# RmSchaffert/ACCV-Lab

Measured on AMD Instinct MI355X. Metric: heatmap frames/sec (1920x1080 fp32, ragged N_obj in [1,128], fused clear+draw), higher is better.
Workload: dtype f32

## Files before the change

### accv-lab_amd/accvlab/_amd_native/__init__.py

```python
from __future__ import annotations

import ctypes
import os

_HERE = os.path.dirname(os.path.abspath(__file__))
NO_HOST_FASTPATH = os.environ.get("ACCV_NO_HOST_FASTPATH", "") not in ("", "0")
LIB_PATH = os.environ.get("ACCV_HIP_LIB") or os.path.join(_HERE, "libaccv_hip.so")

OK = 0
HM_CLEAR = 1
HM_COUNTS_I64 = 2
HM_SMALL_RADII = 4
HM_WRITE_THROUGH = 8
HM_GROUP_BOXES_GIVEN = 16
HM_TILE_ROWS_16 = 32
HM_TILE_ROWS_8 = 64
HM_CALLER_SCALE_ORDER = 256
HM_PLAIN_STORES = 128
HM_POINT_COUNTS_I64 = 512
MP_IDX_I64 = 1
MP_COUNTS_I64 = 2
MP_LABELS_I64 = 4
FL_AVG_NUM_POS = 0
FL_AVG_VALUE = 1
FL_AVG_DEVICE = 2
LSA_MAXIMIZE = 1
LSA_THREADS_64 = 2
LSA_THREADS_1024 = 4
MC_ONE_MINUS_PROB = 0
MC_NEG_PROB = 1
MC_FOCAL = 2
MC_LABELS_I64 = 1
MC_CXCYWH = 2
CR_MAX_MAPS = 8
CR_MAX_CHANNELS = 64
CR_COUNTS_I64 = 1
CR_INDEX_FORM = 2
CR_WEIGHTS_PER_CHANNEL = 4
CR_L1 = 0
CR_SMOOTH_L1 = 2
MF_IDX_I64 = 1
MF_LABELS_I64 = 2
MB_IDX_I64 = 1
MB_CXCYWH = 2
MB_IOU_NONE = 0
MB_IOU = 1
MB_GIOU = 2
MB_MAX_D = 16

_vp = ctypes.c_void_p
_i = ctypes.c_int
_f = ctypes.c_float
_u = ctypes.c_uint
_sz = ctypes.c_size_t
_i64 = ctypes.c_int64
_ll = ctypes.c_longlong
_u64 = ctypes.c_uint64

SIGNATURES = {
    "accv_last_error": (ctypes.c_char_p, []),
    "accv_version": (_i, []),
    "accv_draw_heatmap_last_dispatch": (ctypes.c_char_p, []),
    "accv_draw_heatmap_time_next_launch": (_i, [_vp, _vp]),
    "accv_draw_heatmap_flat_workspace_bytes": (_sz, [_i, _i]),
    "accv_draw_heatmap_flat_f32": (_i, [_vp, _i, _i, _i, _vp, _vp, _vp, _i, _f, _f, _u, _vp, _sz, _vp]),
    "accv_draw_heatmap_batched_f32": (_i, [_vp, _i, _i, _i, _i, _vp, _vp, _vp, _vp, _i, _f, _f, _u, _vp]),
    "accv_fill_f32": (_i, [_vp, _sz, _f, _vp]),
    "accv_draw_heatmap_multiscale_f32": (_i, [_vp, _vp, _vp, _vp, _i, _i, _vp, _vp, _vp, _i, _f, _f, _u, _vp]),
    "accv_draw_heatmap_multiscale_sample_f32": (_i, [_vp, _vp, _vp, _vp, _i, _i, _vp, _vp, _vp, _i, _f, _f, _u,
                                                      _vp, _i, _i, _vp, _i, _vp, _vp, _vp]),
    "accv_draw_points_workspace_bytes": (_sz, [_i, _i]),
    "accv_draw_points_multiscale_f32": (_i, [_vp, _vp, _vp, _vp, _i, _i, _vp, _vp, _i, _i, _f, _f, _u, _vp, _sz, _vp]),
# ... 246 lines not shown
```

### accv-lab_amd/accvlab/draw_heatmap/ops.py

```python
from __future__ import annotations

import ctypes
from typing import Optional

import torch

from .. import _amd_native as _nat

try:
    from . import _dh_host as _dh
except ImportError:
    _dh = None
_native_bound = False


def _native():
    global _native_bound
    if _dh is None or _nat.NO_HOST_FASTPATH:
        return None
    if not _native_bound:
        h = _nat.ctypes_lib()
        addr = lambda name: ctypes.cast(getattr(h, name), ctypes.c_void_p).value
        _dh.bind_native(addr("accv_draw_heatmap_batched_f32"), addr("accv_last_error"))
        _native_bound = True
    return _dh


_FORCED_FLAGS = 0


def _hint_flags(clear: bool, small_radii: bool, write_through: bool, tile_rows) -> int:
    if tile_rows not in (None, 8, 16):
        raise RuntimeError("tile_rows must be None, 8 or 16")
    return (_nat.HM_CLEAR if clear else 0) | (_nat.HM_SMALL_RADII if small_radii else 0) | \
        (0 if write_through is None else _nat.HM_WRITE_THROUGH if write_through else _nat.HM_PLAIN_STORES) | \
        (_nat.HM_TILE_ROWS_16 if tile_rows == 16 else _nat.HM_TILE_ROWS_8 if tile_rows == 8 else 0) | _FORCED_FLAGS


def _one_launch_maps(maps, batch: int, device):
    k = len(maps)
    if not 1 <= k <= 4:
        return None
    ptrs, hs, ws = [], [], []
    for hm in maps:
        if not (isinstance(hm, torch.Tensor) and hm.is_cuda and hm.dtype == torch.float32 and hm.is_contiguous() and
                hm.device == device):
            return None
        shape = hm.shape
        if len(shape) != 3 or shape[0] != batch:
            return None
        ptr = hm.data_ptr()
        if shape[2] % 4 or ptr % 16 or shape[1] * shape[2] * 4 >= (1 << 31):
            return None
        ptrs.append(ptr)
        hs.append(shape[1])
        ws.append(shape[2])
    return (ctypes.c_void_p * k)(*ptrs), (ctypes.c_int * k)(*hs), (ctypes.c_int * k)(*ws)


def _check_maps(maps, batch: int, device, owner: str) -> None:
    for hm in maps:
        _check_input(hm, "heatmap")
        _check_dtype(hm, torch.float32, "heatmap")
        if not (hm.dim() == 3 and hm.size(0) == batch):
            raise RuntimeError("every heatmap must be of shape [batch_size, height, width]")
        if not (hm.device == device):
            raise RuntimeError(f"every heatmap must be on the {owner}' device ({device})")


def _require(cond: bool, msg: str) -> None:
    if not cond:
        raise RuntimeError(msg)


def _check_input(t: torch.Tensor, name: str) -> None:
    if not (isinstance(t, torch.Tensor)):
        raise RuntimeError(f"{name} must be a torch.Tensor")
    if not (t.is_cuda):
        raise RuntimeError(f"{name} must be a CUDA tensor")
    if not (t.is_contiguous()):
        raise RuntimeError(f"{name} must be contiguous")


def _check_dtype(t: torch.Tensor, dtype: torch.dtype, name: str) -> None:
    if not (t.dtype == dtype):
        raise RuntimeError(f"{name}: expected scalar type {dtype} but found {t.dtype}")


def _same_device(ref: torch.Tensor, *others) -> None:
# ... 46 lines not shown
    _check_input(heatmap_idxes, "heatmap_idxes")
    if not (centers.size(0) == radii.size(0)):
        raise RuntimeError("centers and radii must have the same size at dim0")
    if not (centers.size(0) == heatmap_idxes.size(0)):
        raise RuntimeError("centers and heatmap_idxes must have the same size at dim0")
    if not (heatmaps.dim() == 3):
        raise RuntimeError("heatmap must be of shape [num_heatmaps, height, width]")
    if not (centers.dim() == 2 and centers.size(1) == 2):
        raise RuntimeError("centers must be of shape [num_targets, 2]")
    if not (radii.dim() == 1 and heatmap_idxes.dim() == 1):
        raise RuntimeError("radii and heatmap_idxes must be of shape [num_targets]")
    _check_dtype(heatmaps, torch.float32, "heatmap")
    _check_dtype(centers, torch.int32, "centers")
    _check_dtype(radii, torch.int32, "radii")
    _check_dtype(heatmap_idxes, torch.int32, "heatmap_idxes")
    _same_device(heatmaps, ("centers", centers), ("radii", radii), ("heatmap_idxes", heatmap_idxes))

    lib = _nat.lib()
    planes, height, width = heatmaps.shape
    n = centers.size(0)
    if _flat_direct(planes, height, width, n):
        with _nat.device_guard(heatmaps.device):
            dev = heatmaps.device
            count = _device_constant(("count", n, dev), lambda: torch.full((1,), n, dtype=torch.int32, device=dev))
            status = lib.accv_draw_heatmap_batched_f32(
                heatmaps.data_ptr(), 1, planes, height, width, centers.data_ptr(), radii.data_ptr(), count.data_ptr(),
                heatmap_idxes.data_ptr(), n, float(diameter_to_sigma_factor), float(k_scale),
                _hint_flags(clear, small_radii, write_through, tile_rows), _nat.stream_ptr(heatmaps.device))
        _nat.check(status, "draw_heatmap")
        return
    with _nat.device_guard(heatmaps.device):
        ws_bytes = lib.accv_draw_heatmap_flat_workspace_bytes(planes, n)
        ws = torch.empty(ws_bytes, dtype=torch.uint8, device=heatmaps.device)
        status = lib.accv_draw_heatmap_flat_f32(
            heatmaps.data_ptr(), planes, height, width, centers.data_ptr(), radii.data_ptr(),
            heatmap_idxes.data_ptr(), n, float(diameter_to_sigma_factor), float(k_scale),
            _hint_flags(clear, small_radii, write_through, tile_rows), ws.data_ptr(), ws_bytes,
            _nat.stream_ptr(heatmaps.device))
    _nat.check(status, "draw_heatmap")


def draw_heatmap_batched(
    heatmap: torch.Tensor,
    centers,
    radii,
    diameter_to_sigma_factor: float = 6.0,
    k_scale: float = 1.0,
    labels=None,
    *,
    clear: bool = False,
    small_radii: bool = False,
    write_through: Optional[bool] = None,
    tile_rows: Optional[int] = None,
) -> None:
    centers_t = centers.tensor
    radii_t = radii.tensor
    assert centers_t.shape[0] == radii_t.shape[0], "centers and radii must have the same size batch size"
    assert centers_t.shape[1] == radii_t.shape[1], "centers and radii must have the same maximum number of objects"
    counts = centers.sample_sizes
    labels_t: Optional[torch.Tensor] = None
    if labels is not None:
        labels_t = labels.tensor
        assert centers_t.shape[0] == labels_t.shape[0], "centers and labels must have the same size batch size"
        assert centers_t.shape[1] == labels_t.shape[1], \
            "centers and labels must have the same maximum number of objects"

    native = _native()
    if native is not None and isinstance(heatmap, torch.Tensor) and isinstance(counts, torch.Tensor) and \
            native.draw_batched(heatmap, centers_t, radii_t, counts, labels_t, float(diameter_to_sigma_factor), float(k_scale),
                                _hint_flags(clear, small_radii, write_through, tile_rows)):
        return

    if counts.dtype not in (torch.int32, torch.int64):
        counts = counts.to(torch.int64)

    _check_input(heatmap, "heatmap")
    _check_input(centers_t, "centers")
    _check_input(radii_t, "radii")
    _check_input(counts, "nums_targets")
    batch = heatmap.size(0)
    n_max = radii_t.size(1) if radii_t.dim() >= 2 else -1
    _require(batch == radii_t.size(0) and batch == centers_t.size(0) and batch == counts.size(0),
             "batch_size (dim 0) need to be the same for all inputs")
    if not (centers_t.dim() == 3 and centers_t.size(2) == 2):
        raise RuntimeError("centers must be of shape [batch_size, num_targets, 2]")
    if not (radii_t.dim() == 2):
        raise RuntimeError("radii must be of shape [batch_size, num_targets]")
    if not (n_max == centers_t.size(1)):
        raise RuntimeError("maximum number of targets (dim 1) need to be the same centers and radii")
    if not (counts.dim() == 1):
        raise RuntimeError("nums_targets must be of shape [batch_size]")
    _check_dtype(heatmap, torch.float32, "heatmap")
    _check_dtype(centers_t, torch.int32, "centers")
    _check_dtype(radii_t, torch.int32, "radii")
    others = [("centers", centers_t), ("radii", radii_t), ("nums_targets", counts)]
    if labels_t is None:
        if not (heatmap.dim() == 3):
            raise RuntimeError("heatmap must be of shape [batch_size, height, width]")
        num_classes, (height, width) = 0, heatmap.shape[1:]
        labels_ptr = None
    else:
        _check_input(labels_t, "labels")
        if not (heatmap.dim() == 4):
            raise RuntimeError("heatmap must be of shape [batch_size, max_num_classes, height, width]")
        if not (labels_t.dim() == 2):
            raise RuntimeError("labels must be of shape [batch_size, radii.size(1)]")
        _require(labels_t.size(0) == batch and labels_t.size(1) == n_max,
                 "labels shape must be [batch_size, radii.size(1)]")
        _check_dtype(labels_t, torch.int32, "labels")
        num_classes, height, width = heatmap.shape[1:]
        if not (num_classes > 0 or heatmap.numel() == 0):
            raise RuntimeError("class-wise heatmap needs at least one class plane")
        labels_ptr = labels_t.data_ptr()
        others.append(("labels", labels_t))
    _same_device(heatmap, *others)
    if labels_t is not None and num_classes == 0:
        return

    flags = _hint_flags(clear, small_radii, write_through, tile_rows) | \
        (_nat.HM_COUNTS_I64 if counts.dtype == torch.int64 else 0)
    with _nat.device_guard(heatmap.device):
        status = _nat.lib().accv_draw_heatmap_batched_f32(
            heatmap.data_ptr(), batch, num_classes, height, width, centers_t.data_ptr(), radii_t.data_ptr(),
            counts.data_ptr(), labels_ptr, n_max, float(diameter_to_sigma_factor), float(k_scale), flags,
            _nat.stream_ptr(heatmap.device))
    _nat.check(status, "draw_heatmap_batched")


def get_centers_and_radii(centers, bboxes, out_size_factor: float):
    ragged = hasattr(centers, "tensor") and hasattr(centers, "create_with_sample_sizes_like_self")
    c_t = centers.tensor if ragged else centers
    b_t = bboxes.tensor if hasattr(bboxes, "tensor") else bboxes
    _require(c_t.shape[-1] == 2 and b_t.shape[-1] == 4 and c_t.shape[:-1] == b_t.shape[:-1],
             "centers must be [..., 2] and bboxes [..., 4] with equal leading dimensions")
    if c_t.is_cuda:
        if not (b_t.device == c_t.device):
            raise RuntimeError("centers and bboxes must be on the same device")
        c32 = c_t.to(torch.float32).contiguous()
        b32 = b_t.to(torch.float32).contiguous()
        out_c = torch.empty(c32.shape, dtype=torch.int32, device=c32.device)
        out_r = torch.empty(c32.shape[:-1], dtype=torch.int32, device=c32.device)
        with _nat.device_guard(c32.device):
            _nat.check(_nat.lib().accv_heatmap_targets_from_boxes_f32(
                c32.data_ptr(), b32.data_ptr(), out_r.numel(), float(out_size_factor), out_c.data_ptr(),
                out_r.data_ptr(), _nat.stream_ptr(c32.device)), "get_centers_and_radii")
    else:
        d = torch.cat([c_t - b_t[..., :2], b_t[..., 2:] - c_t], dim=-1)
        out_r = torch.ceil(torch.min(d, dim=-1)[0] / out_size_factor).to(torch.int32).clamp_(min=1)
        out_c = (c_t / out_size_factor).to(torch.int32)
    if ragged:
        nu = centers.non_uniform_dim
        return centers.create_with_sample_sizes_like_self(out_c, nu), centers.create_with_sample_sizes_like_self(out_r, nu)
    return out_c, out_r


def draw_heatmap_multiscale(heatmaps, centers, bboxes, out_size_factors, diameter_to_sigma_factor: float = 6.0,
                            k_scale: float = 1.0, *, clear: bool = False) -> None:
    heatmaps = list(heatmaps)
    strides = [float(f) for f in out_size_factors]
    if not (len(heatmaps) == len(strides) and len(heatmaps) >= 1):
        raise RuntimeError("heatmaps and out_size_factors must have the same, non-zero length")
    objects = _box_objects(centers, bboxes)
    batch, dev = objects[0].size(0), objects[0].device
    geometry = _one_launch_maps(heatmaps, batch, dev)
    if geometry is None:
        _check_maps(heatmaps, batch, dev, "centers")
        for hm, f in zip(heatmaps, strides):
            ci, ri = get_centers_and_radii(centers, bboxes, f)
            draw_heatmap_batched(hm, ci, ri, diameter_to_sigma_factor, k_scale, clear=clear)
        return
    _launch_box_maps(geometry, strides, objects, diameter_to_sigma_factor, k_scale, clear)

# ... 43 lines not shown
```

### accv-lab_amd/csrc/draw_heatmap.hip

```cpp
#include <hip/hip_runtime.h>
#include <hip/hip_ext.h>

#include <algorithm>
#include <atomic>
#include <climits>
#include <cstdint>
#include <cstring>
#include <type_traits>

#include "accv_common.h"
#include "polyline_arith.h"

namespace {

constexpr int kWavesPerGroup = 1;
constexpr int kBoxTileR = 8;
constexpr int kCand = 64;
constexpr float kLog2e = 1.4426950408889634f;

struct SplatParams {
    float* hm;
    const int32_t* centers;
    const int32_t* radii;
    const int32_t* labels;
    const void* counts;
    const int32_t* plane_off;
    int H, W;
    int n_max;
    int n_classes;
    int tiles_x, tiles_y;
    long long n_tiles;
    float factor, k;
    int counts_i64;
    int grid3d;
    float dense_area;
    const float* centers_f;
    const float* boxes_f;
    float stride;
    int radius, n_groups;
};

constexpr int kMaxScales = 4;
struct MultiParams {
    SplatParams scale[kMaxScales];
    long long tile_begin[kMaxScales + 1];
    int n_scales;
};

struct __attribute__((aligned(16))) Hit {
    int x, y;
    float c2;
    unsigned box;
};

template <int PX>
struct Vec;
typedef float vfloat4 __attribute__((ext_vector_type(4)));
template <>
struct Vec<4> {
    using type = vfloat4;
};
template <>
struct Vec<1> {
    using type = float;
};

__device__ __forceinline__ float raw_exp2(float x) { return __builtin_amdgcn_exp2f(x); }

__device__ __forceinline__ float max_skip_nan(float acc, float v)
{
    float r;
    asm("v_max_f32 %0, %1, %2" : "=v"(r) : "v"(acc), "v"(v));
    return r;
}

struct TileCtx {
    int tx0, ty0, tx1, ty1;
    long long plane;
    const int2* centers2;
    const int32_t* radii;
    const int32_t* labels;
    const float2* centers_f;
    const float4* boxes_f;
    float4 box0;
    float stride;
    int radius;
    int n, cls;
};
// ... 100 lines not shown
        return Cand{(int)__fdiv_rn(c.x, t.stride), (int)__fdiv_rn(c.y, t.stride), t.radius, 0};
    } else {
        const int2 cxy = t.centers2[cc];
        return Cand{cxy.x, cxy.y, t.radii[cc], t.labels[cc]};
    }
}
__device__ __forceinline__ unsigned long long cull_test(const TileCtx& t, int base, int lane, const Cand& c)
{
    constexpr int kClampXY = 1 << 29, kClampR = 1 << 30;
    const int xc = min(max(c.x, -kClampXY), kClampXY), yc = min(max(c.y, -kClampXY), kClampXY);
    const int rc = min(c.r, kClampR);
    const bool hit = (base + lane < t.n) && (t.cls < 0 || c.label == t.cls) && c.r >= 0 && xc - rc < t.tx1 &&
                     xc + rc >= t.tx0 && yc - rc < t.ty1 && yc + rc >= t.ty0;
    return __ballot(hit);
}
template <int SRC = 0>
__device__ __forceinline__ unsigned long long cull_round(const TileCtx& t, int base, int lane, int& x, int& y, int& r)
{
    const Cand c = cull_load<SRC>(t, base, lane);
    x = c.x;
    y = c.y;
    r = c.r;
    return cull_test(t, base, lane, c);
}

__device__ __forceinline__ float hit_exponent_scale(const SplatParams& p, int r)
{
    const float sigma = (float)(2 * r + 1) / p.factor;
    return kLog2e / (2.0f * sigma * sigma);
}
__device__ __forceinline__ Hit make_hit(const SplatParams& p, const TileCtx& t, int x, int y, int r, float c2);
__device__ __forceinline__ Hit make_hit(const SplatParams& p, const TileCtx& t, int x, int y, int r)
{
    return make_hit(p, t, x, y, r, hit_exponent_scale(p, r));
}
__device__ __forceinline__ Hit make_hit(const SplatParams& p, const TileCtx& t, int x, int y, int r, float c2)
{
    const long long x0 = (long long)x - min(x, r), x1 = (long long)x + min((long long)p.W - x, (long long)r + 1);
    const long long y0 = (long long)y - min(y, r), y1 = (long long)y + min((long long)p.H - y, (long long)r + 1);
    const long long xlo = max(x0, (long long)t.tx0) - t.tx0, xhi = min(x1, (long long)t.tx1) - t.tx0;
    const long long ylo = max(y0, (long long)t.ty0) - t.ty0, yhi = min(y1, (long long)t.ty1) - t.ty0;
    unsigned box = 0;
    if (xhi > xlo && yhi > ylo) box = (unsigned)xlo | ((unsigned)xhi << 8) | ((unsigned)ylo << 16) | ((unsigned)yhi << 24);
    return Hit{x, y, c2, box};
}

__device__ __forceinline__ float max3_skip_nan(float acc, float a, float b)
{
    float r;
    asm("v_max3_f32 %0, %1, %2, %3" : "=v"(r) : "v"(acc), "v"(a), "v"(b));
    return r;
}

template <int PX, int R, bool CLEAR, int SM, int WPG, int SRC>
__device__ __forceinline__ void splat_body(const SplatParams& p, long long linear_group)
{
    constexpr int kWavesPerGroup = WPG;
    constexpr int TW = 32 * PX;
    constexpr int TH = 2 * R;
    static_assert(R % 4 == 0, "row registers are fetched four at a time");

    __shared__ Hit s_hit[kWavesPerGroup][kCand];
    __shared__ __attribute__((aligned(16))) float s_ey[kWavesPerGroup][kCand][TH];

    const int lane = threadIdx.x & 63;
    const int wave = __builtin_amdgcn_readfirstlane(threadIdx.x >> 6);
    TileCtx t;
    if (!locate_tile<TW, TH, kWavesPerGroup>(p, wave, t, linear_group)) return;
    const int tx0 = t.tx0, ty0 = t.ty0, n = t.n;
    const long long plane = t.plane;

    const int sub = lane >> 5;
    const int col0 = tx0 + (lane & 31) * PX;

    float acc[R][PX];
    const float init = CLEAR ? 0.0f : __builtin_nanf("");
#pragma unroll
    for (int i = 0; i < R; ++i)
#pragma unroll
        for (int c = 0; c < PX; ++c) acc[i][c] = init;

    int total_hits = 0;
    float cover = 0.0f;

    for (int base = 0; base < n; base += kCand) {
        int x, y, r;
        const unsigned long long m = cull_round<SRC>(t, base, lane, x, y, r);
        if constexpr (SM == 5) {
            const float dia = (float)(2 * min(max(r, 0), 1 << 20) + 1);
            cover += (base + lane < n) ? dia * dia : 0.0f;
        }
        const bool hit = (m >> lane) & 1ull;
        const int nh = __popcll(m);
        if (nh == 0) continue;
        if constexpr (!CLEAR) {
            if (total_hits == 0 && col0 < p.W) {
                const float* plane_rd = p.hm + (size_t)plane * (size_t)p.H * (size_t)p.W;
#pragma unroll
                for (int i = 0; i < R; ++i) {
                    const int row = ty0 + sub * R + i;
                    if (row < p.H) {
                        if constexpr (PX == 4) {
                            const vfloat4 o = *reinterpret_cast<const vfloat4*>(plane_rd + (size_t)row * p.W + col0);
                            acc[i][0] = o.x;
                            acc[i][1] = o.y;
                            acc[i][2] = o.z;
                            acc[i][3] = o.w;
                        } else {
                            acc[i][0] = plane_rd[(size_t)row * p.W + col0];
                        }
                    }
                }
            }
        }
        if (hit) s_hit[wave][__popcll(m & ((1ull << lane) - 1ull))] = make_hit(p, t, x, y, r);
        __builtin_amdgcn_fence(__ATOMIC_RELEASE, "wavefront");
        __builtin_amdgcn_fence(__ATOMIC_ACQUIRE, "wavefront");

        for (int t = lane; t < nh * TH; t += 64) {
            const int h = t / TH, rr = t % TH;
            const Hit hy = s_hit[wave][h];
            const float d = (float)(ty0 + rr - hy.y);
            const float v = p.k * raw_exp2(-(d * d) * hy.c2);
            const unsigned ylo = (hy.box >> 16) & 255u, yhi = hy.box >> 24;
            s_ey[wave][h][rr] = ((unsigned)rr >= ylo && (unsigned)rr < yhi) ? v : __builtin_nanf("");
        }
        __builtin_amdgcn_fence(__ATOMIC_RELEASE, "wavefront");
        __builtin_amdgcn_fence(__ATOMIC_ACQUIRE, "wavefront");

        const unsigned colr0 = (unsigned)(lane & 31) * PX;
        auto column_factors = [&](const Hit& hx, float (&ex)[PX]) {
            const unsigned xlo = hx.box & 255u, xhi = (hx.box >> 8) & 255u;
#pragma unroll
            for (int c = 0; c < PX; ++c) {
                const float d = (float)(col0 + c - hx.x);
                const float e = raw_exp2(-(d * d) * hx.c2);
                ex[c] = (colr0 + c >= xlo && colr0 + c < xhi) ? e : __builtin_nanf("");
            }
        };
        int h = 0;
        for (; CLEAR && h + 1 < nh; h += 2) {
            float exa[PX], exb[PX];
            column_factors(s_hit[wave][h], exa);
            column_factors(s_hit[wave][h + 1], exb);
#pragma unroll
            for (int q = 0; q < R / 4; ++q) {
                const float4 a4 = *reinterpret_cast<const float4*>(&s_ey[wave][h][sub * R + 4 * q]);
                const float4 b4 = *reinterpret_cast<const float4*>(&s_ey[wave][h + 1][sub * R + 4 * q]);
                const float eya[4] = {a4.x, a4.y, a4.z, a4.w}, eyb[4] = {b4.x, b4.y, b4.z, b4.w};
#pragma unroll
                for (int i = 0; i < 4; ++i)
#pragma unroll
                    for (int c = 0; c < PX; ++c)
                        acc[4 * q + i][c] = max3_skip_nan(acc[4 * q + i][c], exa[c] * eya[i], exb[c] * eyb[i]);
            }
        }
        for (; h < nh; ++h) {
            float ex[PX];
            column_factors(s_hit[wave][h], ex);
#pragma unroll
            for (int q = 0; q < R / 4; ++q) {
                const float4 e4 = *reinterpret_cast<const float4*>(&s_ey[wave][h][sub * R + 4 * q]);
                const float ey[4] = {e4.x, e4.y, e4.z, e4.w};
#pragma unroll
                for (int i = 0; i < 4; ++i)
#pragma unroll
                    for (int c = 0; c < PX; ++c) acc[4 * q + i][c] = max_skip_nan(acc[4 * q + i][c], ex[c] * ey[i]);
            }
        }
        total_hits += nh;
        __builtin_amdgcn_fence(__ATOMIC_RELEASE, "wavefront");
        __builtin_amdgcn_fence(__ATOMIC_ACQUIRE, "wavefront");
    }

    if (!CLEAR && total_hits == 0) return;
    if (col0 >= p.W) return;

    using V = typename Vec<PX>::type;
    float* plane_ptr = p.hm + (size_t)plane * (size_t)p.H * (size_t)p.W;
    bool write_through = SM == 4;
    if constexpr (SM == 5 && PX == 4) {
#pragma unroll
        for (int d = 32; d >= 1; d >>= 1) cover += __shfl_xor(cover, d);
        write_through = cover >= p.dense_area;
    }
#pragma unroll
    for (int i = 0; i < R; ++i) {
        const int row = ty0 + sub * R + i;
        if (row >= p.H) break;
        V* dst = reinterpret_cast<V*>(plane_ptr + (size_t)row * p.W + col0);
        V out;
        if constexpr (PX == 4)
            out = V{acc[i][0], acc[i][1], acc[i][2], acc[i][3]};
        else
            out = acc[i][0];
        if constexpr (SM >= 4 && PX == 4) {
            if (write_through) {
                const auto rsrc = __builtin_amdgcn_make_buffer_rsrc(plane_ptr, 0, (int)((size_t)p.H * p.W * 4), 0x00020000);
                __builtin_amdgcn_raw_buffer_store_b128(out, rsrc, (int)(((size_t)row * p.W + col0) * 4), 0, 18);
            } else {
                *dst = out;
            }
        } else {
            *dst = out;
        }
    }
}

template <int PX, int R, bool CLEAR, int SM, int WPG = kWavesPerGroup>
__global__ __launch_bounds__(WPG * 64) void splat_kernel(const SplatParams p)
{
    splat_body<PX, R, CLEAR, SM, WPG, 0>(p, blockIdx.x);
}

__device__ __forceinline__ int scale_of_group(const MultiParams& mp, long long group, long long& first)
{
    int s = 0;
    first = 0;
#pragma unroll
    for (int i = 1; i < kMaxScales; ++i) {
        const long long begin = mp.tile_begin[i];
        if (group >= begin) {
            s = i;
            first = begin;
        }
    }
    return s;
}
template <typename T>
__device__ __forceinline__ void pin_scalar(T& v)
{
    asm volatile("" : "+s"(v));
}
__device__ __forceinline__ SplatParams preload_params(const SplatParams& src)
{
    SplatParams p = src;
    asm volatile("" ::"s"(p.hm), "s"(p.counts), "s"(p.centers_f), "s"(p.boxes_f));
    pin_scalar(p.H);
    pin_scalar(p.W);
    pin_scalar(p.n_max);
    pin_scalar(p.n_classes);
    pin_scalar(p.tiles_x);
    pin_scalar(p.tiles_y);
    pin_scalar(p.n_tiles);
    pin_scalar(p.factor);
    pin_scalar(p.k);
    pin_scalar(p.counts_i64);
    pin_scalar(p.grid3d);
    pin_scalar(p.dense_area);
    pin_scalar(p.stride);
    pin_scalar(p.radius);
    pin_scalar(p.n_groups);
    return p;
}

template <bool CLEAR, int SM>
__global__ __launch_bounds__(64) void splat_multi_kernel(const MultiParams mp)
{
    long long first;
    const int s = scale_of_group(mp, blockIdx.x, first);
    splat_body<4, kBoxTileR, CLEAR, SM, 1, 1>(mp.scale[s], (long long)blockIdx.x - first);
}

constexpr int kSmallTW = 128, kSmallTH = 16;
constexpr int kSmallLdsW = kSmallTW + 4;
// ... 43 lines not shown
                __hip_atomic_fetch_max(&tile[ylo + py][xlo + px], v, __ATOMIC_RELAXED,
                                       WG_SCOPE ? __HIP_MEMORY_SCOPE_WORKGROUP : __HIP_MEMORY_SCOPE_WAVEFRONT);
            }
        }
    }
    __builtin_amdgcn_fence(__ATOMIC_RELEASE, "wavefront");
    __builtin_amdgcn_fence(__ATOMIC_ACQUIRE, "wavefront");
}
template <bool WG_SCOPE>
__device__ __forceinline__ int splat_round(const SplatParams& p, const TileCtx& t, int lane, unsigned long long m, const Cand& cand,
                                           Hit* __restrict__ hits, SmallTile tile, int rows_hint = 0)
{
    const int nh = __popcll(m);
    int rows = 0;
    if ((m >> lane) & 1ull) {
        const Hit mine = make_hit(p, t, cand.x, cand.y, cand.r);
        hits[__popcll(m & ((1ull << lane) - 1ull))] = mine;
        rows = (int)(mine.box >> 24) - (int)((mine.box >> 16) & 255u);
    }
    if (rows_hint == 0) {
#pragma unroll
        for (int d = 32; d >= 1; d >>= 1) rows = max(rows, __shfl_xor(rows, d));
        rows_hint = max(1, __builtin_amdgcn_readfirstlane(rows));
    }
    walk_hits<WG_SCOPE>(p, t, lane, nh, hits, tile, rows_hint);
    return nh;
}

struct GroupBox {
    float x0, y0, x1, y1;
    bool valid;
};
template <bool FIRST = false>
__device__ __forceinline__ GroupBox load_group_box(const SplatParams& p, const TileCtx& t, int g)
{
    float4 v = FIRST ? t.box0 : t.boxes_f[min(g, p.n_groups - 1)];
    asm volatile("" : "+v"(v.x), "+v"(v.y), "+v"(v.z), "+v"(v.w));
    return GroupBox{v.x, v.y, v.z, v.w, g < p.n_groups && g * kCand < t.n && v.x <= v.z};
}
struct ReachBounds {
    float xlo, xhi, ylo, yhi;
};
__device__ __forceinline__ ReachBounds reach_bounds(const TileCtx& t, int rc, int cx0, int cx1, int cy0, int cy1)
{
    const float r1 = (float)min(rc, 1 << 24) + 2.0f;
    return ReachBounds{((float)cx0 - r1) * t.stride, ((float)cx1 + r1) * t.stride, ((float)cy0 - r1) * t.stride,
                       ((float)cy1 + r1) * t.stride};
}
__device__ __forceinline__ bool group_reaches(const GroupBox& b, const ReachBounds& rb)
{
    return b.valid && b.x1 >= rb.xlo && b.x0 < rb.xhi && b.y1 >= rb.ylo && b.y0 < rb.yhi;
}

constexpr int kDppQuad0 = 0x00, kDppQuad1 = 0x55, kDppQuad2 = 0xAA, kDppQuad3 = 0xFF;
constexpr int kDppRowShr = 0x110;
constexpr int kDppWaveShl1 = 0x130, kDppWaveShr1 = 0x138;
template <int CTRL>
__device__ __forceinline__ float dpp_f(float old, float src)
{
    return __int_as_float(__builtin_amdgcn_update_dpp(__float_as_int(old), __float_as_int(src), CTRL, 0xf, 0xf, false));
}
template <int CTRL>
__device__ __forceinline__ int dpp_i(int old, int src)
{
    return __builtin_amdgcn_update_dpp(old, src, CTRL, 0xf, 0xf, false);
}
__device__ __forceinline__ float2 request_group_samples(const TileCtx& t, int sub_base, int lane)
{
    return t.centers_f[min(sub_base + lane, t.n - 1)];
}
struct PixelScale {
    float stride, inv;
    bool pow2;
};
__device__ __forceinline__ PixelScale pixel_scale(float stride)
{
    const bool pow2 = (__float_as_uint(stride) & 0x007fffffu) == 0u && stride > 1.0e-30f && stride < 1.0e30f;
    return PixelScale{stride, pow2 ? 1.0f / stride : 0.0f, pow2};
}
__device__ __forceinline__ float to_pixels(float x, const PixelScale& ps) { return ps.pow2 ? x * ps.inv : __fdiv_rn(x, ps.stride); }
__device__ __forceinline__ Cand group_candidates(const TileCtx& t, const PixelScale& ps, const float2 c, int lane)
{
    Cand out{(int)to_pixels(c.x, ps), (int)to_pixels(c.y, ps), t.radius, 0};
    if ((c.x != c.x) || (c.y != c.y)) out = Cand{0, 0, -1, 0};
    const int nx = dpp_i<kDppWaveShr1>(0, out.x), ny = dpp_i<kDppWaveShr1>(0, out.y), nr = dpp_i<kDppWaveShr1>(-2, out.r);
    if (lane > 0 && nx == out.x && ny == out.y && nr == out.r) out.r = -1;
    return out;
}

template <int SM>
__device__ __forceinline__ void store_segment(const SplatParams& p, float* plane_ptr, int row, int col0, const vfloat4& v)
{
    if constexpr (SM == 4) {
        const auto rsrc = __builtin_amdgcn_make_buffer_rsrc(plane_ptr, 0, (int)((size_t)p.H * p.W * 4), 0x00020000);
        __builtin_amdgcn_raw_buffer_store_b128(v, rsrc, (int)(((size_t)row * p.W + col0) * 4), 0, 18);
    } else {
        *reinterpret_cast<vfloat4*>(plane_ptr + (size_t)row * p.W + col0) = v;
    }
}

template <bool CLEAR, int SM, int RPW>
__device__ __forceinline__ void write_back_rows(const SplatParams& p, const TileCtx& t, float* plane_ptr, SmallTile tile, int row0,
                                                int lane, int col0)
{
    const float init = CLEAR ? 0.0f : -__builtin_inff();
    constexpr int kBatch = RPW > 4 ? 4 : RPW;
    static_assert(RPW % kBatch == 0, "rows per half-wave come in whole batches");
#pragma unroll
    for (int i0 = 0; i0 < RPW; i0 += kBatch) {
        vfloat4 out[kBatch];
#pragma unroll
        for (int i = 0; i < kBatch; ++i) out[i] = *reinterpret_cast<const vfloat4*>(&tile[row0 + i0 + i][(lane & 31) * 4]);
        if constexpr (CLEAR) {
#pragma unroll
            for (int i = 0; i < kBatch; ++i) {
                const int row = t.ty0 + row0 + i0 + i;
                if (row < p.H) store_segment<SM>(p, plane_ptr, row, col0, out[i]);
            }
        } else {
// ... 736 lines not shown
    const size_t i = (size_t)blockIdx.x * 256 + threadIdx.x;
    if (i < n4) dst[i] = make_float4(value, value, value, value);
}
__global__ void fill_tail_kernel(float* __restrict__ dst, size_t n, float value)
{
    const size_t i = (size_t)blockIdx.x * blockDim.x + threadIdx.x;
    if (i < n) dst[i] = value;
}

template <int PX, int R>
int launch_splat(SplatParams p, long long planes, bool clear, int sm, hipStream_t stream, const LaunchEvents& ev)
{
    p.tiles_x = (p.W + 32 * PX - 1) / (32 * PX);
    p.tiles_y = (p.H + 2 * R - 1) / (2 * R);
    p.n_tiles = planes * p.tiles_x * p.tiles_y;
    if (p.n_tiles == 0) return ACCV_OK;
    const int groups_x = (p.tiles_x + kWavesPerGroup - 1) / kWavesPerGroup;
    dim3 grid, block(kWavesPerGroup * 64);
    p.grid3d = (planes <= 65535 && p.tiles_y <= 65535) ? 1 : 0;
    if (p.grid3d) {
        grid = dim3((unsigned)groups_x, (unsigned)p.tiles_y, (unsigned)planes);
    } else {
        const long long groups = (p.n_tiles + kWavesPerGroup - 1) / kWavesPerGroup;
        if (groups > INT_MAX) return accv::fail(ACCV_EINVAL, "draw_heatmap: %lld tiles exceed the grid limit", p.n_tiles);
        grid = dim3((unsigned)groups);
    }
    if (PX == 1 || (sm == 5 && clear)) sm = 0;
    if (sm == 5) {
        if constexpr (PX == 4) launch_maybe_timed(splat_kernel<PX, R, false, 5>, grid, block, stream, ev, p);
    } else {
        with_variant(clear, sm == 4, [&](auto CL, auto SM) {
            if constexpr (PX == 4 || SM == 0) launch_maybe_timed(splat_kernel<PX, R, CL, SM>, grid, block, stream, ev, p);
        });
    }
    note_dispatch("splat_kernel", PX, R, clear, sm, grid, block);
    return accv::check_launch("draw_heatmap splat kernel");
}

long long compute_units()
{
    static std::atomic<int> cached[64];
    int dev = 0;
    if (hipGetDevice(&dev) != hipSuccess || dev < 0 || dev >= 64) return 0;
    int v = cached[dev].load(std::memory_order_relaxed);
    if (v == 0) {
        int n = 0;
        if (hipDeviceGetAttribute(&n, hipDeviceAttributeMultiprocessorCount, dev) != hipSuccess || n <= 0) return 0;
        cached[dev].store(n, std::memory_order_relaxed);
        v = n;
    }
    return v;
}

int dispatch_splat(SplatParams p, long long planes, bool clear, unsigned flags, hipStream_t stream, const LaunchEvents& ev)
{
    const bool small_hint = (flags & ACCV_HM_SMALL_RADII) != 0;
    const bool vec4 = (p.W % 4 == 0) && ((reinterpret_cast<uintptr_t>(p.hm) & 15u) == 0);
    const bool plane_fits_rsrc = (size_t)p.H * p.W * sizeof(float) < ((size_t)1 << 31);
    int nt;
    if (flags & ACCV_HM_WRITE_THROUGH)
        nt = 4;
    else if (flags & ACCV_HM_PLAIN_STORES)
        nt = 0;
    else
        nt = clear ? 0 : 5;
    if (nt >= 2 && !plane_fits_rsrc) nt = 0;
    p.dense_area = 0.75f * (float)p.H * (float)p.W;
    int rows = (flags & ACCV_HM_TILE_ROWS_16) ? 16 : 8;
    if (!(flags & (ACCV_HM_TILE_ROWS_8 | ACCV_HM_TILE_ROWS_16)) && clear && vec4 && !small_hint) {
        const long long cus = compute_units();
        const long long tx = (p.W + 127) / 128;
        const long long tiles8 = planes * tx * ((p.H + 15) / 16), tiles16 = planes * tx * ((p.H + 31) / 32);
        if (cus > 0 && tiles8 > 24 * cus && tiles16 <= 16 * cus) rows = 16;
    }
    if (!p.labels) p.labels = p.radii;
    if (!vec4) return launch_splat<1, 8>(p, planes, clear, 0, stream, ev);
    if (small_hint) return launch_splat_small(p, planes, clear, nt == 4, stream, ev);
    if (rows == 16) return launch_splat<4, 16>(p, planes, clear, nt, stream, ev);
    return launch_splat<4, 8>(p, planes, clear, nt, stream, ev);
}

int check_common(int h, int w, const char* who)
{
    if (h < 0 || w < 0) return accv::fail(ACCV_EINVAL, "%s: negative heatmap extent %dx%d", who, h, w);
    if (h > (1 << 29) || w > (1 << 29))
        return accv::fail(ACCV_EINVAL, "%s: heatmap extent %dx%d exceeds 2^29 per dimension", who, h, w);
    return ACCV_OK;
}

inline void coarse_scales_first(MultiParams& mp)
{
    std::stable_sort(mp.scale, mp.scale + mp.n_scales,
                     [](const SplatParams& a, const SplatParams& b) { return a.n_tiles < b.n_tiles; });
    long long tiles = 0;
    for (int i = 0; i < mp.n_scales; ++i) {
        mp.tile_begin[i] = tiles;
        tiles += mp.scale[i].n_tiles;
    }
    mp.tile_begin[mp.n_scales] = tiles;
}
inline void seal_tile_prefix(MultiParams& mp)
{
    for (int i = mp.n_scales + 1; i <= kMaxScales; ++i) mp.tile_begin[i] = mp.tile_begin[mp.n_scales];
}

inline int multiscale_store_mode(unsigned flags) { return (flags & ACCV_HM_WRITE_THROUGH) ? 4 : 0; }

constexpr const char* kPerScaleNote = " (use the per-scale calls otherwise)";
long long setup_scales(MultiParams& mp, const SplatParams& proto, float* const* heatmaps, const int* heights, const int* widths,
                       const float* strides, int num_scales, int batch, int tile_h, unsigned flags, const char* who,
                       const char* map_note)
{
    long long tiles = 0;
    int used = 0;
    for (int i = 0; i < num_scales; ++i) {
        if (int rc = check_common(heights[i], widths[i], who)) return rc;
        if (!(strides[i] > 0.0f)) return accv::fail(ACCV_EINVAL, "%s: stride %d is not positive", who, i);
        if (heights[i] == 0 || widths[i] == 0) continue;
        if (!heatmaps[i]) return accv::fail(ACCV_EINVAL, "%s: heatmap %d is null", who, i);
        if (widths[i] % 4 != 0 || (reinterpret_cast<uintptr_t>(heatmaps[i]) & 15u) ||
// ... 467 lines not shown
```

### include/accv_hip.h

```cpp
#ifndef ACCV_HIP_H
#define ACCV_HIP_H

#include <stddef.h>
#include <stdint.h>

#ifdef __cplusplus
extern "C" {
#endif

#define ACCV_OK 0
#define ACCV_EINVAL (-1)
#define ACCV_ELAUNCH (-2)
#define ACCV_EWORKSPACE (-3)
#define ACCV_ERUNTIME (-4)

#define ACCV_HM_CLEAR 1u
#define ACCV_HM_COUNTS_I64 2u
#define ACCV_HM_SMALL_RADII 4u
#define ACCV_HM_WRITE_THROUGH 8u
#define ACCV_HM_GROUP_BOXES_GIVEN 16u

#define ACCV_HM_PLAIN_STORES 128u
#define ACCV_HM_TILE_ROWS_16 32u
#define ACCV_HM_TILE_ROWS_8 64u
#define ACCV_HM_CALLER_SCALE_ORDER 256u

const char* accv_last_error(void);
int accv_version(void);
const char* accv_draw_heatmap_last_dispatch(void);


int accv_draw_heatmap_time_next_launch(void* start_event, void* stop_event);

size_t accv_draw_heatmap_flat_workspace_bytes(int num_planes, int num_objects);
int accv_draw_heatmap_flat_f32(float* heatmaps, int num_planes, int height, int width, const int32_t* centers,
                               const int32_t* radii, const int32_t* heatmap_idxes, int num_objects,
                               float diameter_to_sigma_factor, float k_scale, unsigned flags, void* workspace,
                               size_t workspace_bytes, void* stream);

int accv_draw_heatmap_batched_f32(float* heatmap, int batch, int num_classes, int height, int width,
                                  const int32_t* centers, const int32_t* radii, const void* counts,
                                  const int32_t* labels, int max_num_targets, float diameter_to_sigma_factor,
                                  float k_scale, unsigned flags, void* stream);

int accv_draw_heatmap_multiscale_f32(float* const* heatmaps, const int* heights, const int* widths, const float* strides,
                                     int num_scales, int batch, const float* centers_xy, const float* boxes_xyxy,
                                     const void* counts, int max_num_targets, float diameter_to_sigma_factor,
                                     float k_scale, unsigned flags, void* stream);

int accv_draw_heatmap_multiscale_sample_f32(float* const* heatmaps, const int* heights, const int* widths, const float* strides,
                                            int num_scales, int batch, const float* centers_xy, const float* boxes_xyxy,
                                            const void* counts, int max_num_targets, float diameter_to_sigma_factor,
                                            float k_scale, unsigned flags, const float* polylines_xy, int num_polylines,
                                            int points, const void* point_counts, int num_samples, float* samples,
                                            float* group_boxes, void* stream);

size_t accv_draw_points_workspace_bytes(int batch, int num_points);
int accv_draw_points_multiscale_f32(float* const* heatmaps, const int* heights, const int* widths, const float* strides,
                                    int num_scales, int batch, const float* points_xy, const void* counts, int num_points,
                                    int radius, float diameter_to_sigma_factor, float k_scale, unsigned flags,
                                    void* workspace, size_t workspace_bytes, void* stream);

#define ACCV_HM_POINT_COUNTS_I64 512u
int accv_draw_polylines_fused_applicable(const int* heights, const int* widths, int num_scales, int batch, int lanes,
                                         int points, int num_samples);
int accv_draw_polylines_multiscale_f32(float* const* heatmaps, const int* heights, const int* widths, const float* strides,
                                       int num_scales, int batch, const float* polylines_xy, int lanes, int points,
                                       const void* point_counts, const void* lane_counts, int num_samples, int radius,
                                       float diameter_to_sigma_factor, float k_scale, unsigned flags, void* stream);

int accv_heatmap_targets_from_boxes_f32(const float* centers_xy, const float* boxes_xyxy, long long num_objects,
                                        float stride, int32_t* out_centers, int32_t* out_radii, void* stream);

int accv_heatmap_targets_from_points_f32(const float* points_xy, long long num_points, float stride, int radius,
                                         int32_t* out_centers, int32_t* out_radii, void* stream);


int accv_ragged_gather(const void* src, void* dst, const void* indices, const void* counts, long long batch,
// ... 272 lines not shown
```

Measured before the change: 707,300.

## Prune dominated gaussian splats per tile via wave-level min reduction

Adds a per-tile dominance prune to the splat kernel. When an object's gaussian fully covers the tile, its smallest exponent at the far corner sets a bound, and any candidate whose nearest-point exponent exceeds that bound plus a margin is dropped, because it cannot win the max. This cuts the per-pixel work for overlapping objects, at the cost of extra ballots, DPP reductions and branching in every cull round. The prune is on by default and can be disabled with a new flag.

```diff
diff --git a/accv-lab_amd/accvlab/_amd_native/__init__.py b/accv-lab_amd/accvlab/_amd_native/__init__.py
--- a/accv-lab_amd/accvlab/_amd_native/__init__.py
+++ b/accv-lab_amd/accvlab/_amd_native/__init__.py
@@ -18,6 +18,7 @@
 HM_CALLER_SCALE_ORDER = 256
 HM_PLAIN_STORES = 128
 HM_POINT_COUNTS_I64 = 512
+HM_NO_DOMINANCE_PRUNE = 1024
 MP_IDX_I64 = 1
 MP_COUNTS_I64 = 2
 MP_LABELS_I64 = 4
diff --git a/accv-lab_amd/accvlab/draw_heatmap/ops.py b/accv-lab_amd/accvlab/draw_heatmap/ops.py
--- a/accv-lab_amd/accvlab/draw_heatmap/ops.py
+++ b/accv-lab_amd/accvlab/draw_heatmap/ops.py
@@ -29,12 +29,13 @@
 _FORCED_FLAGS = 0
 
 
-def _hint_flags(clear: bool, small_radii: bool, write_through: bool, tile_rows) -> int:
+def _hint_flags(clear: bool, small_radii: bool, write_through: bool, tile_rows, dominance_prune: bool = True) -> int:
     if tile_rows not in (None, 8, 16):
         raise RuntimeError("tile_rows must be None, 8 or 16")
     return (_nat.HM_CLEAR if clear else 0) | (_nat.HM_SMALL_RADII if small_radii else 0) | \
         (0 if write_through is None else _nat.HM_WRITE_THROUGH if write_through else _nat.HM_PLAIN_STORES) | \
-        (_nat.HM_TILE_ROWS_16 if tile_rows == 16 else _nat.HM_TILE_ROWS_8 if tile_rows == 8 else 0) | _FORCED_FLAGS
+        (_nat.HM_TILE_ROWS_16 if tile_rows == 16 else _nat.HM_TILE_ROWS_8 if tile_rows == 8 else 0) | \
+        (0 if dominance_prune else _nat.HM_NO_DOMINANCE_PRUNE) | _FORCED_FLAGS
 
 
 def _one_launch_maps(maps, batch: int, device):
@@ -187,6 +188,7 @@
     small_radii: bool = False,
     write_through: Optional[bool] = None,
     tile_rows: Optional[int] = None,
+    dominance_prune: bool = True,
 ) -> None:
     centers_t = centers.tensor
     radii_t = radii.tensor
@@ -203,7 +205,7 @@
     native = _native()
     if native is not None and isinstance(heatmap, torch.Tensor) and isinstance(counts, torch.Tensor) and \
             native.draw_batched(heatmap, centers_t, radii_t, counts, labels_t, float(diameter_to_sigma_factor), float(k_scale),
-                                _hint_flags(clear, small_radii, write_through, tile_rows)):
+                                _hint_flags(clear, small_radii, write_through, tile_rows, dominance_prune)):
         return
 
     if counts.dtype not in (torch.int32, torch.int64):
@@ -252,7 +254,7 @@
     if labels_t is not None and num_classes == 0:
         return
 
-    flags = _hint_flags(clear, small_radii, write_through, tile_rows) | \
+    flags = _hint_flags(clear, small_radii, write_through, tile_rows, dominance_prune) | \
         (_nat.HM_COUNTS_I64 if counts.dtype == torch.int64 else 0)
     with _nat.device_guard(heatmap.device):
         status = _nat.lib().accv_draw_heatmap_batched_f32(
diff --git a/accv-lab_amd/csrc/draw_heatmap.hip b/accv-lab_amd/csrc/draw_heatmap.hip
--- a/accv-lab_amd/csrc/draw_heatmap.hip
+++ b/accv-lab_amd/csrc/draw_heatmap.hip
@@ -4,6 +4,7 @@
 #include <algorithm>
 #include <atomic>
 #include <climits>
+#include <cmath>
 #include <cstdint>
 #include <cstring>
 #include <type_traits>
@@ -34,6 +35,7 @@
     int counts_i64;
     int grid3d;
     float dense_area;
+    float prune_limit;
     const float* centers_f;
     const float* boxes_f;
     float stride;
@@ -240,7 +242,52 @@
     return r;
 }
 
-template <int PX, int R, bool CLEAR, int SM, int WPG, int SRC>
+constexpr int kDppQuad0 = 0x00, kDppQuad1 = 0x55, kDppQuad2 = 0xAA, kDppQuad3 = 0xFF;
+constexpr int kDppRowShr = 0x110;
+constexpr int kDppWaveShl1 = 0x130, kDppWaveShr1 = 0x138;
+template <int CTRL>
+__device__ __forceinline__ float dpp_f(float old, float src)
+{
+    return __int_as_float(__builtin_amdgcn_update_dpp(__float_as_int(old), __float_as_int(src), CTRL, 0xf, 0xf, false));
+}
+template <int CTRL>
+__device__ __forceinline__ int dpp_i(int old, int src)
+{
+    return __builtin_amdgcn_update_dpp(old, src, CTRL, 0xf, 0xf, false);
+}
+
+constexpr float kPruneMargin = 0.00390625f;
+constexpr int kDppRowRor = 0x120;
+__device__ __forceinline__ unsigned long long prune_dominated(const SplatParams& p, const TileCtx& t, unsigned long long m, bool hit,
+                                                              int x, int y, int r, const Hit& mine, unsigned& far_bits)
+{
+    constexpr unsigned kSafe = 1u << 29, kInf = 0x7f800000u;
+    const bool ok = hit && (unsigned)x + kSafe <= 2u * kSafe && (unsigned)y + kSafe <= 2u * kSafe && (unsigned)r <= kSafe;
+    const int px = ok ? x : 0, py = ok ? y : 0;
+    const int xlo = mine.box & 255u, xhi = (mine.box >> 8) & 255u, ylo = (mine.box >> 16) & 255u, yhi = mine.box >> 24;
+    const float dxn = (float)max(max(t.tx0 + xlo - px, px - (t.tx0 + xhi - 1)), 0);
+    const float dyn = (float)max(max(t.ty0 + ylo - py, py - (t.ty0 + yhi - 1)), 0);
+    const float dxf = (float)max(px - t.tx0, t.tx1 - 1 - px), dyf = (float)max(py - t.ty0, t.ty1 - 1 - py);
+    const float e_near = ok ? (dxn * dxn + dyn * dyn) * mine.c2 : __builtin_nanf("");
+    const float e_far = (dxf * dxf + dyf * dyf) * mine.c2;
+    const unsigned full_box = (unsigned)(t.tx1 - t.tx0) << 8 | (unsigned)(t.ty1 - t.ty0) << 24;
+    const bool pruner = ok && mine.box == full_box && e_far < p.prune_limit;
+    if (__ballot(pruner)) {
+        int fb = pruner ? __float_as_int(e_far) : (int)kInf;
+        fb = min(fb, dpp_i<kDppRowRor + 8>(fb, fb));
+        fb = min(fb, dpp_i<kDppRowRor + 4>(fb, fb));
+        fb = min(fb, dpp_i<kDppRowRor + 2>(fb, fb));
+        fb = min(fb, dpp_i<kDppRowRor + 1>(fb, fb));
+        const int lo = min(__builtin_amdgcn_readlane(fb, 0), __builtin_amdgcn_readlane(fb, 16));
+        const int hi = min(__builtin_amdgcn_readlane(fb, 32), __builtin_amdgcn_readlane(fb, 48));
+        far_bits = min(far_bits, (unsigned)min(lo, hi));
+    }
+    if (far_bits == kInf) return m;
+    const float limit = __uint_as_float(far_bits) + kPruneMargin;
+    return __ballot(hit && !(e_near > limit));
+}
+
+template <int PX, int R, bool CLEAR, int SM, int WPG, int SRC, bool PRUNE = false>
 __device__ __forceinline__ void splat_body(const SplatParams& p, long long linear_group)
 {
     constexpr int kWavesPerGroup = WPG;
@@ -270,16 +317,17 @@
 
     int total_hits = 0;
     float cover = 0.0f;
+    unsigned far_bits = 0x7f800000u;
 
     for (int base = 0; base < n; base += kCand) {
         int x, y, r;
-        const unsigned long long m = cull_round<SRC>(t, base, lane, x, y, r);
+        unsigned long long m = cull_round<SRC>(t, base, lane, x, y, r);
         if constexpr (SM == 5) {
             const float dia = (float)(2 * min(max(r, 0), 1 << 20) + 1);
             cover += (base + lane < n) ? dia * dia : 0.0f;
         }
-        const bool hit = (m >> lane) & 1ull;
-        const int nh = __popcll(m);
+        bool hit = (m >> lane) & 1ull;
+        int nh = __popcll(m);
         if (nh == 0) continue;
         if constexpr (!CLEAR) {
             if (total_hits == 0 && col0 < p.W) {
@@ -301,7 +349,17 @@
                 }
             }
         }
-        if (hit) s_hit[wave][__popcll(m & ((1ull << lane) - 1ull))] = make_hit(p, t, x, y, r);
+        Hit mine{};
+        if (hit) mine = make_hit(p, t, x, y, r);
+        if constexpr (PRUNE) {
+            if (p.prune_limit > 0.0f && (nh > 1 || far_bits != 0x7f800000u || base + kCand < n)) {
+                m = prune_dominated(p, t, m, hit, x, y, r, mine, far_bits);
+                hit = (m >> lane) & 1ull;
+                nh = __popcll(m);
+                if (nh == 0) continue;
+            }
+        }
+        if (hit) s_hit[wave][__popcll(m & ((1ull << lane) - 1ull))] = mine;
         __builtin_amdgcn_fence(__ATOMIC_RELEASE, "wavefront");
         __builtin_amdgcn_fence(__ATOMIC_ACQUIRE, "wavefront");
 
@@ -398,7 +456,7 @@
 template <int PX, int R, bool CLEAR, int SM, int WPG = kWavesPerGroup>
 __global__ __launch_bounds__(WPG * 64) void splat_kernel(const SplatParams p)
 {
-    splat_body<PX, R, CLEAR, SM, WPG, 0>(p, blockIdx.x);
+    splat_body<PX, R, CLEAR, SM, WPG, 0, true>(p, blockIdx.x);
 }
 
 __device__ __forceinline__ int scale_of_group(const MultiParams& mp, long long group, long long& first)
@@ -548,19 +606,6 @@
     return b.valid && b.x1 >= rb.xlo && b.x0 < rb.xhi && b.y1 >= rb.ylo && b.y0 < rb.yhi;
 }
 
-constexpr int kDppQuad0 = 0x00, kDppQuad1 = 0x55, kDppQuad2 = 0xAA, kDppQuad3 = 0xFF;
-constexpr int kDppRowShr = 0x110;
-constexpr int kDppWaveShl1 = 0x130, kDppWaveShr1 = 0x138;
-template <int CTRL>
-__device__ __forceinline__ float dpp_f(float old, float src)
-{
-    return __int_as_float(__builtin_amdgcn_update_dpp(__float_as_int(old), __float_as_int(src), CTRL, 0xf, 0xf, false));
-}
-template <int CTRL>
-__device__ __forceinline__ int dpp_i(int old, int src)
-{
-    return __builtin_amdgcn_update_dpp(old, src, CTRL, 0xf, 0xf, false);
-}
 __device__ __forceinline__ float2 request_group_samples(const TileCtx& t, int sub_base, int lane)
 {
     return t.centers_f[min(sub_base + lane, t.n - 1)];
@@ -1403,6 +1448,13 @@
     return v;
 }
 
+float prune_limit_for(float k)
+{
+    if (!(k > 0.0f) || !std::isfinite(k)) return 0.0f;
+    const int e = std::ilogb(k);
+    return (float)std::max(0, std::min(120, e + 122));
+}
+
 int dispatch_splat(SplatParams p, long long planes, bool clear, unsigned flags, hipStream_t stream, const LaunchEvents& ev)
 {
     const bool small_hint = (flags & ACCV_HM_SMALL_RADII) != 0;
@@ -1417,6 +1469,7 @@
         nt = clear ? 0 : 5;
     if (nt >= 2 && !plane_fits_rsrc) nt = 0;
     p.dense_area = 0.75f * (float)p.H * (float)p.W;
+    p.prune_limit = (flags & ACCV_HM_NO_DOMINANCE_PRUNE) ? 0.0f : prune_limit_for(p.k);
     int rows = (flags & ACCV_HM_TILE_ROWS_16) ? 16 : 8;
     if (!(flags & (ACCV_HM_TILE_ROWS_8 | ACCV_HM_TILE_ROWS_16)) && clear && vec4 && !small_hint) {
         const long long cus = compute_units();
diff --git a/include/accv_hip.h b/include/accv_hip.h
--- a/include/accv_hip.h
+++ b/include/accv_hip.h
@@ -24,6 +24,7 @@
 #define ACCV_HM_TILE_ROWS_16 32u
 #define ACCV_HM_TILE_ROWS_8 64u
 #define ACCV_HM_CALLER_SCALE_ORDER 256u
+#define ACCV_HM_NO_DOMINANCE_PRUNE 1024u
 
 const char* accv_last_error(void);
 int accv_version(void);
```

Result: no change. 703,500 (-0.5%).
